# alxn3/nbody-llm

Measured on AMD Instinct MI355X. Metric: pairwise_interactions_per_sec, higher is better.
Workload: dtype f32

## Files before the change

### nbody-llm_amd/csrc/kernels.h

```cpp
#pragma once
#include <hip/hip_runtime.h>
#include <cstdint>
#include <vector>

namespace nbody {

struct Tuning {
    int cross_sym = 1;
    int sym_packed = 1;
    int bf_fast_variant = 0;
    int bh_walk_duo = -1;
    int bh_walk_xcd = 1;
    int let_list_div = 4;
    int sym_ipt = 0;
    int sym_wpb = 4;
    int sym_rounds = 1;
    int sym_k = 0;
    int sym_min_bodies = 1024;
    int sym_reduce_split = 1;
    int cross_slots = 3072;
    int cross_ipt = 0;
    int cross_wpb = 4;
    int bh_walk_split = 0;
    int bh_walk_order = 1;
// ... 2 lines not shown
    int bh_walk_variant = 0;
    int bh_walk_lds_block = 1024;
    int bh_hot_cap = 2048;
    int bh_walk_debug = 0;
    int sym_debug = 0;
};
const Tuning& tuning();
struct WalkPlan { int bodies_per_lane; int segments; };
WalkPlan walk_plan(size_t n_order, bool fast_math, int max_segments, float theta2);
void bind_tuning(const Tuning* t);

struct Shard {
    float4* pos_all = nullptr;
    float4* vel = nullptr;
    float4* acc = nullptr;
    int* seg_count = nullptr;
    int* escaped = nullptr;
    unsigned char* keep = nullptr;
    unsigned long long* tile_state = nullptr;
    int* epoch = nullptr;
    int* poison = nullptr;
    int* ids = nullptr;
    unsigned long long* inter = nullptr;
    int n_seg = 1;
    int seg_cap = 0;
    int my_seg = 0;
    float4* own_pos() const { return pos_all + size_t(my_seg) * seg_cap; }
    int* own_count() const { return seg_count + my_seg; }
};

struct BoundsF {
    float lo[3];
    float hi[3];
};

void launch_aos_to_soa(hipStream_t s, const float* aos, int stride_f, int n, float4* pos, float4* vel, float4* acc);
void launch_soa_to_aos(hipStream_t s, float* aos, int stride_f, int n, const float4* pos, const float4* vel, const float4* acc);

void launch_drift_half(hipStream_t s, const Shard& sh, int n_upper, float dt, BoundsF b);
void launch_compact(hipStream_t s, const Shard& sh, int n_upper);
void launch_kick_drift(hipStream_t s, const Shard& sh, int n_upper, float dt);

void launch_bf_forces_strict(hipStream_t s, const Shard& sh, int n_upper, float g, float g_soft2);
void launch_bf_forces_fast(hipStream_t s, const Shard& sh, int n_upper, float g, float g_soft2);

struct SymPlan {
    int ipt = 8;
    int A = 0;
    int K = 0;
    int wpb = 16;
    int res_combine = 0;
    int k_res = 0;
    int sym_sets = 0;
    int n_planes = 0;
    int k_os = 0;
    size_t n_pad = 0;
    size_t plane_stride = 0;
    std::vector<int> bounds;
};
SymPlan make_sym_plan(int n_upper);
int sym_bodies_per_lane(size_t n);
uint64_t sym_main_pairs(const SymPlan& p, size_t n);
void launch_bf_sym_main(hipStream_t s, const Shard& sh, const SymPlan& p, const int* d_bounds, float4* planes,
                        int n_upper, float g_soft2);
void launch_bf_os(hipStream_t s, const Shard& sh, int A, int K, float4* planes, size_t plane_stride, float g_soft2);
void launch_bf_sym_tail(hipStream_t s, const Shard& sh, const SymPlan& p, float4* planes, int n_upper, float g,
                        float g_soft2, const float* kick_dt);

struct CrossPartners {
    static constexpr int kMax = 8;
    int n = 0;
    int seg[kMax];
    int c0[kMax], c1[kMax];
    int a0[kMax], a1[kMax];
};
struct CrossPlan {
    static constexpr int kMaxPlanes = 256;
    int ipt = 8;
    int A = 0;
    CrossPartners parts;
    int n_recv = 0;
    int recv_from[CrossPartners::kMax];
    int k_res = 0;
    std::vector<int4> slices;
};
CrossPlan make_cross_plan(int rank, int world, int seg_cap, int n_own_upper);
void launch_bf_cross(hipStream_t s, const Shard& sh, const CrossPlan& p, const int4* d_slices, float4* res_planes,
                     float4* xplanes, float4* send, size_t plane_stride, float g_soft2);

constexpr int kMaxSplit = 64, kMaxAnc = 192;
constexpr size_t kSplitInts = size_t(kMaxSplit) + 1 + kMaxSplit + size_t(kMaxSplit) * kMaxAnc;
struct TreeDev {
    const float4* nodes = nullptr;
    int n_nodes = 0;
    const int* order = nullptr;
    int n_order = 0;
    int n_split = 1;
    const int* split_first = nullptr;
    const int* split_anc = nullptr;
    const int* split_n_anc = nullptr;
    float4* split_planes = nullptr;
    size_t split_stride = 0;
    float4* nested_stack = nullptr;
    size_t nested_stride = 0;
    float4* walk = nullptr;
    float4* hot = nullptr;
    int* unified = nullptr;
    int* hot_info = nullptr;
    int hot_cap = 0;
    int hot_threshold = 0;
    const int* poison = nullptr;
    const int* n_order_dev = nullptr;
    int store_work = 0;
    float4* bfs = nullptr;
    void* bfs_ws = nullptr;
    size_t bfs_cap = 0;
};
struct TreeDevWork {
    const unsigned long long* keys = nullptr;
    const signed char* delta = nullptr;
// ... 59 lines not shown
```

### nbody-llm_amd/csrc/kernels_bf_sym.hip

```cpp
#include "kernels.h"
#include "bf_pair.h"

#include <algorithm>

namespace nbody {

namespace {

#ifdef NBODY_TUNING
__device__ unsigned long long nbody_sym_stamps[3 * 8192];
#endif

}

template <int IPT>
__device__ __forceinline__ void sym_rest_wave(const float4* __restrict__ pos, int n, int A, int group, int slice,
                                              int n_slices, float& ax, float& ay, float& az, float eps2);

template <int IPT, int NW>
__device__ __forceinline__ void sym_rest_block(const float4* __restrict__ pos, int n, int A, int group,
                                               float4* __restrict__ plane, float eps2, float (*red)[3][64]);

template <int IPT, int WPB, int DBG = 0, bool PK = false>
__global__ __launch_bounds__(WPB * 64) void k_bf_sym(const float4* __restrict__ pos, const int* __restrict__ count,
                                                     int A, int K, const int* __restrict__ bounds, int sym_sets,
                                                     float4* __restrict__ planes, size_t plane_stride, float eps2,
                                                     int res_combine) {
    const int lane = threadIdx.x & 63;
    const int wslot = __builtin_amdgcn_readfirstlane(threadIdx.x >> 6);
    const int n_main_blocks = (A * K + WPB - 1) / WPB;
    if (int(blockIdx.x) >= n_main_blocks) {
        __shared__ float red[WPB - 1][3][64];
        sym_rest_block<IPT, WPB>(pos, *count, A, blockIdx.x - n_main_blocks,
                                 planes + size_t(sym_sets + (res_combine ? K / WPB : K)) * plane_stride, eps2, red);
        return;
    }
    const int gw = blockIdx.x * WPB + (wslot & 3) * (WPB / 4) + (wslot >> 2);
    if (gw >= A * K) return;
    const int a = gw / K;
    const int part = gw - a * K;
    const int n = *count;
    const int Cn = A * IPT;
    const int k0 = bounds[part], k1 = bounds[part + 1];
    const int src_lane = ((lane + 63) & 63) * 4;
    const int src_lane2 = ((lane + 62) & 63) * 4;
    float eps2v = eps2;
    asm volatile("" : "+v"(eps2v));

    float xi[IPT], yi[IPT], zi[IPT], mi[IPT], axi[IPT], ayi[IPT], azi[IPT];
#pragma unroll
    for (int q = 0; q < IPT; ++q) {
        const int i = (a * IPT + q) * 64 + lane;
        const float4 p = (i < n) ? pos[i] : make_float4(PAD_POS, PAD_POS, PAD_POS, 0.f);
        xi[q] = p.x; yi[q] = p.y; zi[q] = p.z; mi[q] = p.w;
        axi[q] = ayi[q] = azi[q] = 0.f;
    }

    auto chunk_of = [&](int k) {
        int c = (a + 1) * IPT + k;
        if (c >= Cn) c -= Cn;
        return c;
    };
    auto load_chunk = [&](int k) {
        const int j = chunk_of(k) * 64 + lane;
        return (j < n) ? pos[j] : make_float4(PAD_POS, PAD_POS, PAD_POS, 0.f);
    };

    [[maybe_unused]] unsigned long long t_beg = 0, r_beg = 0;
    if (DBG & 4) { t_beg = __builtin_amdgcn_s_memtime(); r_beg = __builtin_amdgcn_s_memrealtime(); }
    float4 nxt = (k0 < k1) ? load_chunk(k0) : make_float4(0.f, 0.f, 0.f, 0.f);
    v2f xi2[IPT / 2], yi2[IPT / 2], zi2[IPT / 2], mi2[IPT / 2], axi2[IPT / 2], ayi2[IPT / 2], azi2[IPT / 2];
    if (PK) {
        pack_pairs<IPT>(xi, xi2); pack_pairs<IPT>(yi, yi2); pack_pairs<IPT>(zi, zi2); pack_pairs<IPT>(mi, mi2);
        pack_pairs<IPT>(axi, axi2); pack_pairs<IPT>(ayi, ayi2); pack_pairs<IPT>(azi, azi2);
    }
    for (int k = k0; k < k1; ++k) {
        float xj = nxt.x, yj = nxt.y, zj = nxt.z, mj = nxt.w;
        float axj = 0.f, ayj = 0.f, azj = 0.f;
        v2f axj2 = {0.f, 0.f}, ayj2 = {0.f, 0.f}, azj2 = {0.f, 0.f};
        if (k + 1 < k1) nxt = load_chunk(k + 1);
        switch ((4 * (k1 - k) - 1) / (k1 - k0)) {
            case 3: __builtin_amdgcn_s_setprio(3); break;
            case 2: __builtin_amdgcn_s_setprio(2); break;
            case 1: __builtin_amdgcn_s_setprio(1); break;
            default: __builtin_amdgcn_s_setprio(0); break;
        }
        if (PK) {
            for (int s = 0; s < 64; s += 2) {
                const float x1 = rotl(xj, src_lane), y1 = rotl(yj, src_lane), z1 = rotl(zj, src_lane), m1 = rotl(mj, src_lane);
                pair_evals_pk<IPT / 2, DBG>(xi2, yi2, zi2, mi2, axi2, ayi2, azi2, xj, yj, zj, mj, axj2, ayj2, azj2, eps2v);
                axj2.x = rotl(axj2.x, src_lane); ayj2.x = rotl(ayj2.x, src_lane); azj2.x = rotl(azj2.x, src_lane);
                axj2.y = rotl(axj2.y, src_lane); ayj2.y = rotl(ayj2.y, src_lane); azj2.y = rotl(azj2.y, src_lane);
                xj = rotl(x1, src_lane); yj = rotl(y1, src_lane); zj = rotl(z1, src_lane); mj = rotl(m1, src_lane);
                pair_evals_pk<IPT / 2, DBG>(xi2, yi2, zi2, mi2, axi2, ayi2, azi2, x1, y1, z1, m1, axj2, ayj2, azj2, eps2v);
                axj2.x = rotl(axj2.x, src_lane); ayj2.x = rotl(ayj2.x, src_lane); azj2.x = rotl(azj2.x, src_lane);
                axj2.y = rotl(axj2.y, src_lane); ayj2.y = rotl(ayj2.y, src_lane); azj2.y = rotl(azj2.y, src_lane);
            }
        } else {
            float x1 = rotl(xj, src_lane), y1 = rotl(yj, src_lane), z1 = rotl(zj, src_lane), m1 = rotl(mj, src_lane);
#pragma unroll 2
            for (int s = 0; s < 64; ++s) {
                const float x2 = rotl(xj, src_lane2), y2 = rotl(yj, src_lane2), z2 = rotl(zj, src_lane2), m2 = rotl(mj, src_lane2);
                pair_evals<IPT, DBG>(xi, yi, zi, mi, axi, ayi, azi, xj, yj, zj, mj, axj, ayj, azj, eps2v);
                axj = rotl(axj, src_lane); ayj = rotl(ayj, src_lane); azj = rotl(azj, src_lane);
                xj = x1; yj = y1; zj = z1; mj = m1;
                x1 = x2; y1 = y2; z1 = z2; m1 = m2;
            }
        }
        if (PK) { axj = axj2.x + axj2.y; ayj = ayj2.x + ayj2.y; azj = azj2.x + azj2.y; }
        const int d = k / IPT + 1;
        planes[size_t(d - 1) * plane_stride + size_t(chunk_of(k)) * 64 + lane] = make_float4(axj, ayj, azj, 0.f);
    }
    if (PK) { unpack_pairs<IPT>(axi2, axi); unpack_pairs<IPT>(ayi2, ayi); unpack_pairs<IPT>(azi2, azi); }

#ifdef NBODY_TUNING
    if (DBG & 4) {
        const unsigned long long t_end = __builtin_amdgcn_s_memtime(), r_end = __builtin_amdgcn_s_memrealtime();
        if (lane == 0 && gw < 8192) {
            nbody_sym_stamps[gw * 3 + 0] = t_end - t_beg;
            nbody_sym_stamps[gw * 3 + 1] = r_end - r_beg;
            const unsigned hw = __builtin_amdgcn_s_getreg((4 ) | (0 << 6) | (31 << 11));
            const unsigned xcc = __builtin_amdgcn_s_getreg((20 ) | (0 << 6) | (31 << 11));
            nbody_sym_stamps[gw * 3 + 2] = (unsigned long long)(k1 - k0) | ((unsigned long long)hw << 16) | ((unsigned long long)(xcc & 0xF) << 48);
        }
    }
#endif
    if (res_combine) {
        __shared__ float comb[WPB - 1][3 * IPT][64];
        const int first_part = (part / WPB) * WPB;
        const int rel = part - first_part;
        if (rel > 0) {
#pragma unroll
            for (int q = 0; q < IPT; ++q) {
                comb[rel - 1][3 * q + 0][lane] = axi[q];
                comb[rel - 1][3 * q + 1][lane] = ayi[q];
                comb[rel - 1][3 * q + 2][lane] = azi[q];
            }
        }
        __syncthreads();
        if (rel == 0) {
            float4* __restrict__ out = planes + size_t(sym_sets + part / WPB) * plane_stride;
#pragma unroll
            for (int q = 0; q < IPT; ++q) {
                float sx = axi[q], sy = ayi[q], sz = azi[q];
                for (int w = 0; w < WPB - 1; ++w) { sx += comb[w][3 * q + 0][lane]; sy += comb[w][3 * q + 1][lane]; sz += comb[w][3 * q + 2][lane]; }
                out[size_t(a * IPT + q) * 64 + lane] = make_float4(sx, sy, sz, 0.f);
            }
        }
        return;
    }
    float4* __restrict__ out = planes + size_t(sym_sets + part) * plane_stride;
#pragma unroll
    for (int q = 0; q < IPT; ++q) out[size_t(a * IPT + q) * 64 + lane] = make_float4(axi[q], ayi[q], azi[q], 0.f);
}

template <int IPT, int WPB, bool PK>
__global__ __launch_bounds__(WPB * 64) void k_bf_os(const float4* __restrict__ pos_all,
                                                    const int* __restrict__ seg_count, int n_seg, int seg_cap,
                                                    int my_seg, int A, int K, float4* __restrict__ planes,
                                                    size_t plane_stride, float eps2) {
    __shared__ float4 stage[WPB][2][64];
    const int lane = threadIdx.x & 63;
    const int wslot = __builtin_amdgcn_readfirstlane(threadIdx.x >> 6);
    const int gw = blockIdx.x * WPB + (wslot & 3) * (WPB / 4) + (wslot >> 2);
    if (gw >= A * K) return;
    const int a = gw / K, part = gw - a * K;
    const int n_own = seg_count[my_seg];
    const float4* __restrict__ own = pos_all + size_t(my_seg) * seg_cap;
    float eps2v = eps2;
    asm volatile("" : "+v"(eps2v));

    float xi[IPT], yi[IPT], zi[IPT], mi[IPT], axi[IPT], ayi[IPT], azi[IPT];
#pragma unroll
    for (int q = 0; q < IPT; ++q) {
        const int i = (a * IPT + q) * 64 + lane;
        const float4 p = (i < n_own) ? own[i] : make_float4(PAD_POS, PAD_POS, PAD_POS, 0.f);
        xi[q] = p.x; yi[q] = p.y; zi[q] = p.z; mi[q] = p.w;
        axi[q] = ayi[q] = azi[q] = 0.f;
    }
    long long R = 0;
    for (int s = 0; s < n_seg; ++s) if (s != my_seg) R += seg_count[s];
    const long long r0 = R * part / K, r1 = R * (part + 1) / K;
    long long seg_first = 0;
    float dummy_x = 0.f, dummy_y = 0.f, dummy_z = 0.f;
    v2f dummy2 = {0.f, 0.f};
    v2f xi2[IPT / 2], yi2[IPT / 2], zi2[IPT / 2], mi2[IPT / 2], axi2[IPT / 2], ayi2[IPT / 2], azi2[IPT / 2];
    if (PK) {
        pack_pairs<IPT>(xi, xi2); pack_pairs<IPT>(yi, yi2); pack_pairs<IPT>(zi, zi2); pack_pairs<IPT>(mi, mi2);
        pack_pairs<IPT>(axi, axi2); pack_pairs<IPT>(ayi, ayi2); pack_pairs<IPT>(azi, azi2);
    }
    for (int s = 0; s < n_seg; ++s) {
        if (s == my_seg) continue;
        const int ns = seg_count[s];
        const long long lo = r0 > seg_first ? r0 : seg_first;
        const long long hi = r1 < seg_first + ns ? r1 : seg_first + ns;
        const float4* __restrict__ ps = pos_all + size_t(s) * seg_cap - seg_first;
        int buf = 0;
        if (lo < hi) {
            const long long j = lo + lane;
            stage[wslot][0][lane] = (j < hi) ? ps[j] : make_float4(PAD_POS, PAD_POS, PAD_POS, 0.f);
        }
        for (long long c0 = lo; c0 < hi; c0 += 64) {
            const long long jn = c0 + 64 + lane;
            float4 nxt = make_float4(PAD_POS, PAD_POS, PAD_POS, 0.f);
            if (c0 + 64 < hi && jn < hi) nxt = ps[jn];
            const int cnt = int(hi - c0 < 64 ? hi - c0 : 64);
            switch (int((4 * (r1 - c0) - 1) / (r1 - r0))) {
                case 3: __builtin_amdgcn_s_setprio(3); break;
                case 2: __builtin_amdgcn_s_setprio(2); break;
                case 1: __builtin_amdgcn_s_setprio(1); break;
                default: __builtin_amdgcn_s_setprio(0); break;
            }
            float4 pj = stage[wslot][buf][0];
            for (int t = 0; t < cnt; ++t) {
                const float4 pn = stage[wslot][buf][(t + 1) & 63];
                if (PK)
                    pair_evals_pk<IPT / 2, 0, false>(xi2, yi2, zi2, mi2, axi2, ayi2, azi2, pj.x, pj.y, pj.z, pj.w, dummy2,
                                                     dummy2, dummy2, eps2v);
                else
                    pair_evals<IPT, 0, false>(xi, yi, zi, mi, axi, ayi, azi, pj.x, pj.y, pj.z, pj.w, dummy_x, dummy_y,
                                              dummy_z, eps2v);
                pj = pn;
            }
            buf ^= 1;
            stage[wslot][buf][lane] = nxt;
        }
        seg_first += ns;
    }
    if (PK) { unpack_pairs<IPT>(axi2, axi); unpack_pairs<IPT>(ayi2, ayi); unpack_pairs<IPT>(azi2, azi); }
    float4* __restrict__ out = planes + size_t(part) * plane_stride;
#pragma unroll
    for (int q = 0; q < IPT; ++q) out[size_t(a * IPT + q) * 64 + lane] = make_float4(axi[q], ayi[q], azi[q], 0.f);
}

template <int IPT>
__device__ __forceinline__ void sym_rest_wave(const float4* __restrict__ pos, int n, int A, int group, int slice,
                                              int n_slices, float& ax, float& ay, float& az, float eps2) {
    constexpr int SET = 64 * IPT;
    const int lane = threadIdx.x & 63;
    const int i = group * 64 + lane;
    const int a = (group * 64) / SET;
    const float4 pi = (i < n) ? pos[i] : make_float4(PAD_POS, PAD_POS, PAD_POS, 0.f);
    ax = ay = az = 0.f;
    const int n_win = (A % 2 == 0 && A > 1) ? 2 : 1;
    for (int w = 0; w < n_win; ++w) {
        int set = (w == 0) ? a : a + A / 2;
        if (set >= A) set -= A;
        const int j0 = set * SET + SET * slice / n_slices;
        const int j1 = min(n, set * SET + SET * (slice + 1) / n_slices);
#pragma unroll 8
        for (int j = j0; j < j1; ++j) {
            const float4 pj = pos[j];
            const float dx = pj.x - pi.x, dy = pj.y - pi.y, dz = pj.z - pi.z;
            const float r2 = __builtin_fmaf(dz, dz, __builtin_fmaf(dy, dy, __builtin_fmaf(dx, dx, eps2)));
            const float rinv = __builtin_amdgcn_rsqf(r2);
            float sj = pj.w * ((rinv * rinv) * rinv);
            sj = (j == i) ? 0.f : sj;
            ax = __builtin_fmaf(dx, sj, ax);
            ay = __builtin_fmaf(dy, sj, ay);
            az = __builtin_fmaf(dz, sj, az);
        }
    }
}

template <int IPT, int NW>
__device__ __forceinline__ void sym_rest_block(const float4* __restrict__ pos, int n, int A, int group,
                                               float4* __restrict__ plane, float eps2, float (*red)[3][64]) {
    const int lane = threadIdx.x & 63;
    const int wv = __builtin_amdgcn_readfirstlane(threadIdx.x >> 6);
    float ax, ay, az;
    sym_rest_wave<IPT>(pos, n, A, group, wv, NW, ax, ay, az, eps2);
    if (wv > 0) { red[wv - 1][0][lane] = ax; red[wv - 1][1][lane] = ay; red[wv - 1][2][lane] = az; }
    __syncthreads();
    if (wv == 0) {
#pragma unroll
        for (int w = 0; w < NW - 1; ++w) { ax += red[w][0][lane]; ay += red[w][1][lane]; az += red[w][2][lane]; }
        plane[group * 64 + lane] = make_float4(ax, ay, az, 0.f);
    }
}

template <int IPT>
__global__ __launch_bounds__(512) void k_bf_sym_rest(const float4* __restrict__ pos, const int* __restrict__ count,
                                                     int A, float4* __restrict__ plane, float eps2) {
    __shared__ float red[7][3][64];
    sym_rest_block<IPT, 8>(pos, *count, A, blockIdx.x, plane, eps2, red);
}

template <bool KICK>
__global__ __launch_bounds__(256) void k_bf_sym_reduce(const float4* __restrict__ planes, int n_planes,
                                                       size_t plane_stride, const int* __restrict__ count, float g,
                                                       float4* __restrict__ acc, float4* __restrict__ pos,
                                                       float4* __restrict__ vel, float dt, const int* __restrict__ seg_count,
                                                       int n_seg, unsigned long long* __restrict__ inter) {
    const int i = blockIdx.x * 256 + threadIdx.x;
    if (inter && i == 0) {
        long long tot = 0;
        for (int s = 0; s < n_seg; ++s) tot += seg_count[s];
        if (tot > 0) atomicAdd(inter, (unsigned long long)(*count) * (unsigned long long)(tot - 1));
    }
    if (i >= *count) return;
    float sx = 0.f, sy = 0.f, sz = 0.f, cx = 0.f, cy = 0.f, cz = 0.f;
    for (int p = 0; p < n_planes; ++p) {
        const float4 v = planes[size_t(p) * plane_stride + i];
        const float yx = v.x - cx, yy = v.y - cy, yz = v.z - cz;
        const float tx = sx + yx, ty = sy + yy, tz = sz + yz;
        cx = (tx - sx) - yx; cy = (ty - sy) - yy; cz = (tz - sz) - yz;
        sx = tx; sy = ty; sz = tz;
    }
    const float4 a = make_float4(g * sx, g * sy, g * sz, 0.f);
    acc[i] = a;
    if (KICK) {
        float4 p = pos[i], v = vel[i];
        v.x += a.x * dt; v.y += a.y * dt; v.z += a.z * dt;
        p.x += (v.x * 0.5f) * dt; p.y += (v.y * 0.5f) * dt; p.z += (v.z * 0.5f) * dt;
        vel[i] = v;
        pos[i] = p;
    }
}

template <bool KICK, int Q>
__global__ __launch_bounds__(64 * Q) void k_bf_sym_reduce_split(const float4* __restrict__ planes, int n_planes, size_t plane_stride,
                                                                const int* __restrict__ count, float g, float4* __restrict__ acc,
                                                                float4* __restrict__ pos, float4* __restrict__ vel, float dt,
                                                                const int* __restrict__ seg_count, int n_seg,
                                                                unsigned long long* __restrict__ inter) {
    __shared__ float part[Q][3][64];
    const int lane = threadIdx.x & 63, q = threadIdx.x >> 6;
    const int i = blockIdx.x * 64 + lane;
    if (inter && blockIdx.x == 0 && threadIdx.x == 0) {
        long long tot = 0;
        for (int s = 0; s < n_seg; ++s) tot += seg_count[s];
        if (tot > 0) atomicAdd(inter, (unsigned long long)(*count) * (unsigned long long)(tot - 1));
    }
    const int n = *count;
    float sx = 0.f, sy = 0.f, sz = 0.f, cx = 0.f, cy = 0.f, cz = 0.f;
    if (i < n) {
        const int p0 = int((long long)n_planes * q / Q), p1 = int((long long)n_planes * (q + 1) / Q);
        for (int p = p0; p < p1; ++p) {
            const float4 v = planes[size_t(p) * plane_stride + i];
            const float yx = v.x - cx, yy = v.y - cy, yz = v.z - cz;
            const float tx = sx + yx, ty = sy + yy, tz = sz + yz;
            cx = (tx - sx) - yx; cy = (ty - sy) - yy; cz = (tz - sz) - yz;
            sx = tx; sy = ty; sz = tz;
        }
    }
    part[q][0][lane] = sx; part[q][1][lane] = sy; part[q][2][lane] = sz;
    __syncthreads();
    if (q != 0 || i >= n) return;
    sx = sy = sz = cx = cy = cz = 0.f;
    for (int w = 0; w < Q; ++w) {
        const float yx = part[w][0][lane] - cx, yy = part[w][1][lane] - cy, yz = part[w][2][lane] - cz;
        const float tx = sx + yx, ty = sy + yy, tz = sz + yz;
        cx = (tx - sx) - yx; cy = (ty - sy) - yy; cz = (tz - sz) - yz;
        sx = tx; sy = ty; sz = tz;
    }
    const float4 a = make_float4(g * sx, g * sy, g * sz, 0.f);
    acc[i] = a;
    if (KICK) {
        float4 p = pos[i], v = vel[i];
        v.x += a.x * dt; v.y += a.y * dt; v.z += a.z * dt;
        p.x += (v.x * 0.5f) * dt; p.y += (v.y * 0.5f) * dt; p.z += (v.z * 0.5f) * dt;
        vel[i] = v;
        pos[i] = p;
    }
}

}
#ifdef NBODY_TUNING
namespace nbody { int read_sym_stamps(unsigned long long* out, int n_waves); }
extern "C" int nbody_sym_read_stamps(unsigned long long* out, int n_waves) { return nbody::read_sym_stamps(out, n_waves); }
#endif
namespace nbody {

int sym_bodies_per_lane(size_t n) {
    const Tuning& t = tuning();
    if (!t.sym_packed || t.sym_wpb != 4 || t.sym_ipt == 8) return 8;
    if (t.sym_ipt == 4) return 4;
    return n <= 10240 ? 4 : 8;
}

SymPlan make_sym_plan(int n_upper) {
    SymPlan p;
    const int IPT = sym_bodies_per_lane(size_t(n_upper));
    p.ipt = IPT;
    p.A = (n_upper + 64 * IPT - 1) / (64 * IPT);
    p.sym_sets = (p.A + 1) / 2 - 1;
    const int L = IPT * p.sym_sets;
    const int want = tuning().sym_wpb;
    p.wpb = want == 8 ? 8 : want == 12 ? 12 : want == 16 ? 16 : 4;
    int K = 1;
    if (p.wpb == 4) {
        K = L <= 100 ? L : L <= 160 ? (L + 1) / 2 : 64;
    } else {
        const int resident_wgs_per_cu = (p.wpb == 8) ? 2 : 1;
        const int slots = 256 * resident_wgs_per_cu * p.wpb;
        double best = 0.0;
        const int k_hi = std::min(126, std::min(L, std::max(1, slots * std::max(1, tuning().sym_rounds) * 4 / p.A)));
        for (int k = 1; k <= k_hi; ++k) {
            const long long waves = (long long)p.A * k;
            const long long rounds = (waves + slots - 1) / slots;
            if (rounds > 4 * std::max(1, tuning().sym_rounds) && k > 1) break;
            const double fill = double(waves) / double(rounds * slots);
            const double even = (L % k == 0) ? 1.0 : double(L / k) / double(L / k + 1);
            const double per_wave = double(L) / k / (double(L) / k + 0.3);
            if (fill * even * per_wave > best + 1e-9) { best = fill * even * per_wave; K = k; }
        }
    }
    if (tuning().sym_k > 0) K = std::min(126, tuning().sym_k);
    if (K > L) K = L;
    if (K < 1) K = 1;
    p.K = K;
    p.res_combine = (K % p.wpb == 0) ? 1 : 0;
    p.k_res = p.res_combine ? K / p.wpb : K;
    p.n_planes = p.sym_sets + p.k_res + 1;
    p.n_pad = size_t(p.A) * 64 * IPT;
    p.plane_stride = p.n_pad;
    p.bounds.resize(K + 1);
    for (int part = 0; part <= K; ++part) p.bounds[part] = int((long long)L * part / K);
    return p;
}

#ifdef NBODY_TUNING
int read_sym_stamps(unsigned long long* out, int n_waves) {
    return hipMemcpyFromSymbol(out, HIP_SYMBOL(nbody_sym_stamps), sizeof(unsigned long long) * 3 * n_waves) == hipSuccess ? 0 : -1;
}
#endif

uint64_t sym_main_pairs(const SymPlan& p, size_t n) {
    const size_t set = size_t(64) * p.ipt;
    auto size_of = [&](int a) { size_t lo = size_t(a) * set; return lo >= n ? size_t(0) : std::min(set, n - lo); };
    uint64_t pairs = 0;
    for (int a = 0; a < p.A; ++a)
        for (int d = 1; d <= p.sym_sets; ++d) pairs += uint64_t(size_of(a)) * uint64_t(size_of((a + d) % p.A));
    return pairs;
}

void launch_bf_sym_main(hipStream_t s, const Shard& sh, const SymPlan& p, const int* d_bounds, float4* planes,
                        int n_upper, float g_soft2) {
    if (n_upper <= 0 || p.sym_sets <= 0) return;
    const int main_blocks = (p.A * p.K + p.wpb - 1) / p.wpb;
    const int rest_blocks = int(p.n_pad / 64);
    const dim3 grid(main_blocks + rest_blocks), block(p.wpb * 64);
#define SYM_LAUNCH(WPB, DBG) hipLaunchKernelGGL((k_bf_sym<8, WPB, DBG, PKV>), grid, block, 0, s, sh.own_pos(), sh.own_count(), p.A, p.K, d_bounds, p.sym_sets, planes, p.plane_stride, g_soft2, p.res_combine)
#ifdef NBODY_TUNING
    const int dbg = tuning().sym_debug;
#else
    constexpr int dbg = 0;
#endif
    if (p.ipt == 4) {
        hipLaunchKernelGGL((k_bf_sym<4, 4, 0, true>), grid, block, 0, s, sh.own_pos(), sh.own_count(), p.A, p.K, d_bounds, p.sym_sets, planes, p.plane_stride, g_soft2, p.res_combine);
        return;
    }
    if (tuning().sym_packed) {
        constexpr bool PKV = true;
        if (dbg == 4) {
#ifdef NBODY_TUNING
            if (p.wpb == 12) SYM_LAUNCH(12, 4); else if (p.wpb == 8) SYM_LAUNCH(8, 4); else if (p.wpb == 4) SYM_LAUNCH(4, 4); else SYM_LAUNCH(16, 4);
#endif
        } else {
            if (p.wpb == 12) SYM_LAUNCH(12, 0); else if (p.wpb == 8) SYM_LAUNCH(8, 0); else if (p.wpb == 4) SYM_LAUNCH(4, 0); else SYM_LAUNCH(16, 0);
        }
    } else {
        constexpr bool PKV = false;
        if (dbg >= 4 && dbg <= 7) {
#ifdef NBODY_TUNING
            if (dbg == 4) { if (p.wpb == 12) SYM_LAUNCH(12, 4); else if (p.wpb == 8) SYM_LAUNCH(8, 4); else if (p.wpb == 4) SYM_LAUNCH(4, 4); else SYM_LAUNCH(16, 4); }
            else if (dbg == 5) SYM_LAUNCH(16, 5);
            else if (dbg == 6) SYM_LAUNCH(16, 6);
            else SYM_LAUNCH(16, 7);
#endif
        } else {
            if (p.wpb == 12) SYM_LAUNCH(12, 0); else if (p.wpb == 8) SYM_LAUNCH(8, 0); else if (p.wpb == 4) SYM_LAUNCH(4, 0); else SYM_LAUNCH(16, 0);
        }
    }
#undef SYM_LAUNCH
}

void launch_bf_os(hipStream_t s, const Shard& sh, int A, int K, float4* planes, size_t plane_stride, float g_soft2) {
    if (A <= 0 || K <= 0) return;
    const int wpb = 12;
    if (tuning().sym_packed)
        hipLaunchKernelGGL((k_bf_os<8, 12, true>), dim3((A * K + wpb - 1) / wpb), dim3(wpb * 64), 0, s, sh.pos_all,
                           sh.seg_count, sh.n_seg, sh.seg_cap, sh.my_seg, A, K, planes, plane_stride, g_soft2);
    else
        hipLaunchKernelGGL((k_bf_os<8, 12, false>), dim3((A * K + wpb - 1) / wpb), dim3(wpb * 64), 0, s, sh.pos_all,
                           sh.seg_count, sh.n_seg, sh.seg_cap, sh.my_seg, A, K, planes, plane_stride, g_soft2);
}

void launch_bf_sym_tail(hipStream_t s, const Shard& sh, const SymPlan& p, float4* planes, int n_upper, float g,
                        float g_soft2, const float* kick_dt) {
    if (n_upper <= 0) return;
    if (p.sym_sets == 0) {
        float4* resident0 = planes + size_t(p.sym_sets) * p.plane_stride;
        (void)hipMemsetAsync(resident0, 0, size_t(p.k_res) * p.plane_stride * sizeof(float4), s);
        if (p.ipt == 4)
            hipLaunchKernelGGL(k_bf_sym_rest<4>, dim3(int(p.n_pad / 64)), dim3(512), 0, s, sh.own_pos(),
                               sh.own_count(), p.A, planes + size_t(p.sym_sets + p.k_res) * p.plane_stride, g_soft2);
        else
        hipLaunchKernelGGL(k_bf_sym_rest<8>, dim3(int(p.n_pad / 64)), dim3(512), 0, s, sh.own_pos(),
                           sh.own_count(), p.A, planes + size_t(p.sym_sets + p.k_res) * p.plane_stride, g_soft2);
    }
    const float dt = kick_dt ? *kick_dt : 0.f;
#define REDUCE_ARGS planes, p.n_planes, p.plane_stride, sh.own_count(), g, sh.acc, sh.own_pos(), sh.vel, dt, sh.seg_count, sh.n_seg, sh.inter
    if (tuning().sym_reduce_split && p.n_planes >= 16) {
        const dim3 grid((n_upper + 63) / 64);
        if (n_upper <= 16384) {
            if (kick_dt) hipLaunchKernelGGL((k_bf_sym_reduce_split<true, 16>), grid, dim3(1024), 0, s, REDUCE_ARGS);
            else hipLaunchKernelGGL((k_bf_sym_reduce_split<false, 16>), grid, dim3(1024), 0, s, REDUCE_ARGS);
        } else {
            if (kick_dt) hipLaunchKernelGGL((k_bf_sym_reduce_split<true, 4>), grid, dim3(256), 0, s, REDUCE_ARGS);
            else hipLaunchKernelGGL((k_bf_sym_reduce_split<false, 4>), grid, dim3(256), 0, s, REDUCE_ARGS);
        }
    } else {
        const dim3 grid((n_upper + 255) / 256);
        if (kick_dt) hipLaunchKernelGGL(k_bf_sym_reduce<true>, grid, dim3(256), 0, s, REDUCE_ARGS);
        else hipLaunchKernelGGL(k_bf_sym_reduce<false>, grid, dim3(256), 0, s, REDUCE_ARGS);
    }
#undef REDUCE_ARGS
}

}
```

### nbody-llm_amd/csrc/nbody_api.cpp

```cpp
#include "nbody_handle.h"
#include "nbody_f64.h"
#include "nbody_let.h"

#include <algorithm>
#include <chrono>
#include <cmath>
#include <cstdio>
#include <cstdlib>
#include <cstring>
#include <memory>
#include <string>
#include <thread>
#include <vector>


static thread_local std::string g_create_err;

int fail(NbodyHandle* h, int code, const std::string& msg) {
    if (h) h->err = msg; else g_create_err = msg;
    return code;
}

namespace {

// ... 555 lines not shown
        }
        if (rest.empty()) {
            h->host_tree_once = true;
            return NBODY_OK;
        }
        h->elapsed = rest[0].elapsed_before;
        h->stats.steps -= rest.size();
        h->host_tree_once = true;
        int rc = sync_count(h);
        if (rc) return rc;
        rc = step_end(h, rest[0].dt);
        if (rc) return rc;
        for (size_t k = 1; k < rest.size(); ++k) {
            rc = step_impl(h, rest[k].dt);
            if (rc) return rc;
        }
    }
    return fail(h, NBODY_ERR_INVALID, "resolve_async did not converge");
}

int partials_begin(NbodyHandle* h) {
    if (!(h->cross_on && h->tail_pending) || h->cross.parts.n + h->cross.n_recv == 0) return NBODY_OK;
    if (!h->comm_ready) return fail(h, NBODY_ERR_COMM, "world_size > 1 but nbody_comm_init has not been called");
    const nbody::CrossPlan& c = h->cross;
    const size_t S = h->sym_plan.plane_stride;
    const size_t bytes = size_t(h->sh.seg_cap) * sizeof(float4);
    HIP_TRY(h, hipEventRecord(h->ev_partials_ready, h->stream));
    HIP_TRY(h, hipStreamWaitEvent(h->comm_stream, h->ev_partials_ready, 0));
    TP_TRY(h, h->tp->group_begin());
    for (int i = 0; i < c.parts.n; ++i)
        TP_TRY(h, h->tp->send(h->d_send + size_t(i) * S, bytes, c.parts.seg[i], h->comm_stream));
    for (int i = 0; i < c.n_recv; ++i)
        TP_TRY(h, h->tp->recv(h->d_planes + size_t(h->recv_plane0 + i) * S, bytes, c.recv_from[i], h->comm_stream));
    TP_TRY(h, h->tp->group_end());
    HIP_TRY(h, hipEventRecord(h->ev_partials_done, h->comm_stream));
    h->partials_in_flight = true;
    return NBODY_OK;
}

int partials_wait(NbodyHandle* h) {
    if (!h->partials_in_flight) return NBODY_OK;
    HIP_TRY(h, hipStreamWaitEvent(h->stream, h->ev_partials_done, 0));
    h->partials_in_flight = false;
    return NBODY_OK;
}

int forces_begin(NbodyHandle* h) {
    return h->cfg.method == NBODY_BARNES_HUT ? bh_forces(h) : bf_forces(h);
}

int forces_finish(NbodyHandle* h) {
    if (!h->tail_pending) return NBODY_OK;
    h->tail_pending = false;
    const float eps2 = h->g_soft * h->g_soft;
    nbody::launch_bf_sym_tail(h->stream, h->sh, h->sym_plan, h->d_planes, int(h->n_local), h->g, eps2,
                              h->kick_pending ? &h->kick_dt : nullptr);
    h->kick_pending = false;
    HIP_TRY(h, hipGetLastError());
    return NBODY_OK;
}

int forces(NbodyHandle* h) {
    int rc = forces_begin(h);
    if (rc) return rc;
    rc = partials_begin(h);
    if (rc) return rc;
    rc = partials_wait(h);
    if (rc) return rc;
    return forces_finish(h);
}

int step_begin(NbodyHandle* h, float dt) {
    if (!h->bounds_set) return fail(h, NBODY_ERR_INVALID, "nbody_set_bounds has not been called");
    nbody::launch_drift_half(h->stream, h->sh, int(h->n_local), dt, h->bnd);
    nbody::launch_compact(h->stream, h->sh, int(h->n_local));
    h->count_dirty = true;
    HIP_TRY(h, hipGetLastError());
    return NBODY_OK;
}

int step_forces(NbodyHandle* h, float dt) {
    h->kick_pending = true;
    h->kick_dt = dt;
    int rc = forces_begin(h);
    if (rc) { h->kick_pending = false; h->tail_pending = false; }
    return rc;
}

int step_finish(NbodyHandle* h, float dt) {
    int rc = forces_finish(h);
    if (rc) { h->kick_pending = false; return rc; }
    if (h->kick_pending) nbody::launch_kick_drift(h->stream, h->sh, int(h->n_local), dt);
    h->kick_pending = false;
    HIP_TRY(h, hipGetLastError());
    if (h->ev_pending.size() >= 4096) {
        rc = drain_events(h);
        if (rc) return rc;
    }
    h->elapsed += dt;
    h->stats.steps += 1;
    return NBODY_OK;
}

int step_end(NbodyHandle* h, float dt) {
    int rc = step_forces(h, dt);
    if (rc) return rc;
    rc = partials_begin(h);
    if (rc) return rc;
// ... 1008 lines not shown
```

Measured before the change: 5553 billion.

## Fold diagonal and half-distance chunks into symmetric traversal, add per-lane intra-chunk kernel

Replaces the non-symmetric 'rest' pass, which evaluated the diagonal set and the antipodal set with full one-sided pairs, with symmetric traversal items. The diagonal chunk uses a 32-step rotate with a half-lane final step, and the antipodal set is split across halves. A new small kernel computes intra-lane pairs among each lane's IPT bodies. Work is balanced over 'units', and planes are laid out via n_trav. This removes roughly the redundant half of the rest-pass interactions, at the cost of more index logic and extra planes. Pair accounting now reports n(n-1)/2.

Measured after the change: 5574 billion, median of 6. No clear change (+0.4%).

```diff
diff --git a/nbody-llm_amd/csrc/kernels.h b/nbody-llm_amd/csrc/kernels.h
--- a/nbody-llm_amd/csrc/kernels.h
+++ b/nbody-llm_amd/csrc/kernels.h
@@ -78,6 +78,7 @@
     int res_combine = 0;
     int k_res = 0;
     int sym_sets = 0;
+    int n_trav = 0;
     int n_planes = 0;
     int k_os = 0;
     size_t n_pad = 0;
@@ -91,7 +92,7 @@
                         int n_upper, float g_soft2);
 void launch_bf_os(hipStream_t s, const Shard& sh, int A, int K, float4* planes, size_t plane_stride, float g_soft2);
 void launch_bf_sym_tail(hipStream_t s, const Shard& sh, const SymPlan& p, float4* planes, int n_upper, float g,
-                        float g_soft2, const float* kick_dt);
+                        const float* kick_dt);
 
 struct CrossPartners {
     static constexpr int kMax = 8;
diff --git a/nbody-llm_amd/csrc/kernels_bf_sym.hip b/nbody-llm_amd/csrc/kernels_bf_sym.hip
--- a/nbody-llm_amd/csrc/kernels_bf_sym.hip
+++ b/nbody-llm_amd/csrc/kernels_bf_sym.hip
@@ -13,34 +13,71 @@
 
 }
 
+template <int IPT, int DBG>
+__device__ __forceinline__ void sym_step_pk(const v2f (&xi)[IPT / 2], const v2f (&yi)[IPT / 2], const v2f (&zi)[IPT / 2],
+                                            const v2f (&mi)[IPT / 2], v2f (&axi)[IPT / 2], v2f (&ayi)[IPT / 2],
+                                            v2f (&azi)[IPT / 2], float xj, float yj, float zj, float mj, v2f& axj,
+                                            v2f& ayj, v2f& azj, float eps2) {
+    constexpr int G = (IPT / 2 <= 6) ? IPT / 2 : 4;
+    static_assert((IPT / 2) % G == 0, "resident pairs must split into whole groups");
+#pragma unroll
+    for (int g = 0; g < IPT / 2; g += G) {
+        typedef v2f grp[G];
+        pair_evals_pk<G, DBG>(*reinterpret_cast<const grp*>(xi + g), *reinterpret_cast<const grp*>(yi + g),
+                              *reinterpret_cast<const grp*>(zi + g), *reinterpret_cast<const grp*>(mi + g),
+                              *reinterpret_cast<grp*>(axi + g), *reinterpret_cast<grp*>(ayi + g), *reinterpret_cast<grp*>(azi + g),
+                              xj, yj, zj, mj, axj, ayj, azj, eps2);
+    }
+}
+
 template <int IPT>
-__device__ __forceinline__ void sym_rest_wave(const float4* __restrict__ pos, int n, int A, int group, int slice,
-                                              int n_slices, float& ax, float& ay, float& az, float eps2);
-
-template <int IPT, int NW>
-__device__ __forceinline__ void sym_rest_block(const float4* __restrict__ pos, int n, int A, int group,
-                                               float4* __restrict__ plane, float eps2, float (*red)[3][64]);
+__global__ __launch_bounds__(256) void k_bf_sym_lanes(const float4* __restrict__ pos, const int* __restrict__ count,
+                                                      int A, float4* __restrict__ plane, float eps2) {
+    const int lane = threadIdx.x & 63;
+    const int a = blockIdx.x * 4 + (threadIdx.x >> 6);
+    if (a >= A) return;
+    const int n = *count;
+    float x[IPT], y[IPT], z[IPT], m[IPT], ax[IPT], ay[IPT], az[IPT];
+#pragma unroll
+    for (int q = 0; q < IPT; ++q) {
+        const int i = (a * IPT + q) * 64 + lane;
+        const float4 p = (i < n) ? pos[i] : make_float4(PAD_POS, PAD_POS, PAD_POS, 0.f);
+        x[q] = p.x; y[q] = p.y; z[q] = p.z; m[q] = p.w;
+        ax[q] = ay[q] = az[q] = 0.f;
+    }
+#pragma unroll
+    for (int r = 1; r < IPT; ++r) {
+#pragma unroll
+        for (int q = 0; q < r; ++q) {
+            const float dx = x[r] - x[q], dy = y[r] - y[q], dz = z[r] - z[q];
+            const float r2 = __builtin_fmaf(dz, dz, __builtin_fmaf(dy, dy, __builtin_fmaf(dx, dx, eps2)));
+            const float ri = __builtin_amdgcn_rsqf(r2);
+            const float r3 = (ri * ri) * ri;
+            const float sr = m[r] * r3, sq = m[q] * r3;
+            ax[q] = __builtin_fmaf(dx, sr, ax[q]); ax[r] = __builtin_fmaf(-dx, sq, ax[r]);
+            ay[q] = __builtin_fmaf(dy, sr, ay[q]); ay[r] = __builtin_fmaf(-dy, sq, ay[r]);
+            az[q] = __builtin_fmaf(dz, sr, az[q]); az[r] = __builtin_fmaf(-dz, sq, az[r]);
+            __builtin_amdgcn_sched_barrier(0);
+        }
+    }
+#pragma unroll
+    for (int q = 0; q < IPT; ++q) plane[size_t(a * IPT + q) * 64 + lane] = make_float4(ax[q], ay[q], az[q], 0.f);
+}
 
 template <int IPT, int WPB, int DBG = 0, bool PK = false>
 __global__ __launch_bounds__(WPB * 64) void k_bf_sym(const float4* __restrict__ pos, const int* __restrict__ count,
-                                                     int A, int K, const int* __restrict__ bounds, int sym_sets,
+                                                     int A, int K, const int* __restrict__ bounds, int sym_sets, int n_trav,
                                                      float4* __restrict__ planes, size_t plane_stride, float eps2,
                                                      int res_combine) {
     const int lane = threadIdx.x & 63;
     const int wslot = __builtin_amdgcn_readfirstlane(threadIdx.x >> 6);
-    const int n_main_blocks = (A * K + WPB - 1) / WPB;
-    if (int(blockIdx.x) >= n_main_blocks) {
-        __shared__ float red[WPB - 1][3][64];
-        sym_rest_block<IPT, WPB>(pos, *count, A, blockIdx.x - n_main_blocks,
-                                 planes + size_t(sym_sets + (res_combine ? K / WPB : K)) * plane_stride, eps2, red);
-        return;
-    }
     const int gw = blockIdx.x * WPB + (wslot & 3) * (WPB / 4) + (wslot >> 2);
     if (gw >= A * K) return;
     const int a = gw / K;
     const int part = gw - a * K;
     const int n = *count;
     const int Cn = A * IPT;
+    const int L = IPT * sym_sets;
     const int k0 = bounds[part], k1 = bounds[part + 1];
     const int src_lane = ((lane + 63) & 63) * 4;
     const int src_lane2 = ((lane + 62) & 63) * 4;
@@ -56,29 +93,43 @@
         axi[q] = ayi[q] = azi[q] = 0.f;
     }
 
-    auto chunk_of = [&](int k) {
-        int c = (a + 1) * IPT + k;
-        if (c >= Cn) c -= Cn;
-        return c;
+    auto item_of = [&](int k, int& c, int& s0, int& kind, int& pl) {
+        if (k < L) {
+            c = (a + 1) * IPT + k;
+            if (c >= Cn) c -= Cn;
+            s0 = 0; kind = 0; pl = k / IPT;
+        } else if (k < L + IPT) {
+            c = a * IPT + (k - L); s0 = 1; kind = 1; pl = sym_sets;
+        } else {
+            int b = a + A / 2;
+            if (b >= A) b -= A;
+            c = b * IPT + (k - L - IPT); s0 = (a < A / 2) ? 0 : 1; kind = 2; pl = sym_sets + 1;
+        }
     };
-    auto load_chunk = [&](int k) {
-        const int j = chunk_of(k) * 64 + lane;
+    auto load_item = [&](int k) {
+        int c, s0, kind, pl;
+        item_of(k, c, s0, kind, pl);
+        const int j = c * 64 + ((lane - s0) & 63);
         return (j < n) ? pos[j] : make_float4(PAD_POS, PAD_POS, PAD_POS, 0.f);
     };
 
     [[maybe_unused]] unsigned long long t_beg = 0, r_beg = 0;
     if (DBG & 4) { t_beg = __builtin_amdgcn_s_memtime(); r_beg = __builtin_amdgcn_s_memrealtime(); }
-    float4 nxt = (k0 < k1) ? load_chunk(k0) : make_float4(0.f, 0.f, 0.f, 0.f);
+    float4 nxt = (k0 < k1) ? load_item(k0) : make_float4(0.f, 0.f, 0.f, 0.f);
     v2f xi2[IPT / 2], yi2[IPT / 2], zi2[IPT / 2], mi2[IPT / 2], axi2[IPT / 2], ayi2[IPT / 2], azi2[IPT / 2];
     if (PK) {
         pack_pairs<IPT>(xi, xi2); pack_pairs<IPT>(yi, yi2); pack_pairs<IPT>(zi, zi2); pack_pairs<IPT>(mi, mi2);
         pack_pairs<IPT>(axi, axi2); pack_pairs<IPT>(ayi, ayi2); pack_pairs<IPT>(azi, azi2);
     }
+    const bool low_half = lane < 32;
     for (int k = k0; k < k1; ++k) {
+        int c, s0, kind, pl;
+        item_of(k, c, s0, kind, pl);
+        const int n_steps = kind == 0 ? 64 : 32;
         float xj = nxt.x, yj = nxt.y, zj = nxt.z, mj = nxt.w;
         float axj = 0.f, ayj = 0.f, azj = 0.f;
         v2f axj2 = {0.f, 0.f}, ayj2 = {0.f, 0.f}, azj2 = {0.f, 0.f};
-        if (k + 1 < k1) nxt = load_chunk(k + 1);
+        if (k + 1 < k1) nxt = load_item(k + 1);
         switch ((4 * (k1 - k) - 1) / (k1 - k0)) {
             case 3: __builtin_amdgcn_s_setprio(3); break;
             case 2: __builtin_amdgcn_s_setprio(2); break;
@@ -86,33 +137,49 @@
             default: __builtin_amdgcn_s_setprio(0); break;
         }
         if (PK) {
-            for (int s = 0; s < 64; s += 2) {
+            const int n_it = n_steps / 2 - (kind == 1 ? 1 : 0);
+            for (int it = 0; it < n_it; ++it) {
                 const float x1 = rotl(xj, src_lane), y1 = rotl(yj, src_lane), z1 = rotl(zj, src_lane), m1 = rotl(mj, src_lane);
-                pair_evals_pk<IPT / 2, DBG>(xi2, yi2, zi2, mi2, axi2, ayi2, azi2, xj, yj, zj, mj, axj2, ayj2, azj2, eps2v);
+                sym_step_pk<IPT, DBG>(xi2, yi2, zi2, mi2, axi2, ayi2, azi2, xj, yj, zj, mj, axj2, ayj2, azj2, eps2v);
                 axj2.x = rotl(axj2.x, src_lane); ayj2.x = rotl(ayj2.x, src_lane); azj2.x = rotl(azj2.x, src_lane);
                 axj2.y = rotl(axj2.y, src_lane); ayj2.y = rotl(ayj2.y, src_lane); azj2.y = rotl(azj2.y, src_lane);
                 xj = rotl(x1, src_lane); yj = rotl(y1, src_lane); zj = rotl(z1, src_lane); mj = rotl(m1, src_lane);
-                pair_evals_pk<IPT / 2, DBG>(xi2, yi2, zi2, mi2, axi2, ayi2, azi2, x1, y1, z1, m1, axj2, ayj2, azj2, eps2v);
+                sym_step_pk<IPT, DBG>(xi2, yi2, zi2, mi2, axi2, ayi2, azi2, x1, y1, z1, m1, axj2, ayj2, azj2, eps2v);
                 axj2.x = rotl(axj2.x, src_lane); ayj2.x = rotl(ayj2.x, src_lane); azj2.x = rotl(azj2.x, src_lane);
                 axj2.y = rotl(axj2.y, src_lane); ayj2.y = rotl(ayj2.y, src_lane); azj2.y = rotl(azj2.y, src_lane);
             }
+            if (kind == 1) {
+                const float x1 = rotl(xj, src_lane), y1 = rotl(yj, src_lane), z1 = rotl(zj, src_lane), m1 = rotl(mj, src_lane);
+                sym_step_pk<IPT, DBG>(xi2, yi2, zi2, mi2, axi2, ayi2, azi2, xj, yj, zj, mj, axj2, ayj2, azj2, eps2v);
+                axj2.x = rotl(axj2.x, src_lane); ayj2.x = rotl(ayj2.x, src_lane); azj2.x = rotl(azj2.x, src_lane);
+                axj2.y = rotl(axj2.y, src_lane); ayj2.y = rotl(ayj2.y, src_lane); azj2.y = rotl(azj2.y, src_lane);
+                if (low_half) sym_step_pk<IPT, DBG>(xi2, yi2, zi2, mi2, axi2, ayi2, azi2, x1, y1, z1, m1, axj2, ayj2, azj2, eps2v);
+                axj2.x = rotl(axj2.x, src_lane); ayj2.x = rotl(ayj2.x, src_lane); azj2.x = rotl(azj2.x, src_lane);
+                axj2.y = rotl(axj2.y, src_lane); ayj2.y = rotl(ayj2.y, src_lane); azj2.y = rotl(azj2.y, src_lane);
+            }
         } else {
             float x1 = rotl(xj, src_lane), y1 = rotl(yj, src_lane), z1 = rotl(zj, src_lane), m1 = rotl(mj, src_lane);
-#pragma unroll 2
-            for (int s = 0; s < 64; ++s) {
+            auto step = [&]() {
                 const float x2 = rotl(xj, src_lane2), y2 = rotl(yj, src_lane2), z2 = rotl(zj, src_lane2), m2 = rotl(mj, src_lane2);
                 pair_evals<IPT, DBG>(xi, yi, zi, mi, axi, ayi, azi, xj, yj, zj, mj, axj, ayj, azj, eps2v);
                 axj = rotl(axj, src_lane); ayj = rotl(ayj, src_lane); azj = rotl(azj, src_lane);
                 xj = x1; yj = y1; zj = z1; mj = m1;
                 x1 = x2; y1 = y2; z1 = z2; m1 = m2;
+            };
+            for (int s = 0; s < n_steps / 2 - 1; ++s) { step(); step(); }
+            step();
+            if (kind == 1) {
+                if (low_half) pair_evals<IPT, DBG>(xi, yi, zi, mi, axi, ayi, azi, xj, yj, zj, mj, axj, ayj, azj, eps2v);
+                axj = rotl(axj, src_lane); ayj = rotl(ayj, src_lane); azj = rotl(azj, src_lane);
+            } else {
+                step();
             }
         }
         if (PK) { axj = axj2.x + axj2.y; ayj = ayj2.x + ayj2.y; azj = azj2.x + azj2.y; }
-        const int d = k / IPT + 1;
-        planes[size_t(d - 1) * plane_stride + size_t(chunk_of(k)) * 64 + lane] = make_float4(axj, ayj, azj, 0.f);
+        const int row = c * 64 + ((lane - s0 - n_steps) & 63);
+        planes[size_t(pl) * plane_stride + size_t(row)] = make_float4(axj, ayj, azj, 0.f);
     }
     if (PK) { unpack_pairs<IPT>(axi2, axi); unpack_pairs<IPT>(ayi2, ayi); unpack_pairs<IPT>(azi2, azi); }
-
 #ifdef NBODY_TUNING
     if (DBG & 4) {
         const unsigned long long t_end = __builtin_amdgcn_s_memtime(), r_end = __builtin_amdgcn_s_memrealtime();
@@ -139,7 +206,7 @@
         }
         __syncthreads();
         if (rel == 0) {
-            float4* __restrict__ out = planes + size_t(sym_sets + part / WPB) * plane_stride;
+            float4* __restrict__ out = planes + size_t(n_trav + part / WPB) * plane_stride;
 #pragma unroll
             for (int q = 0; q < IPT; ++q) {
                 float sx = axi[q], sy = ayi[q], sz = azi[q];
@@ -149,7 +216,7 @@
         }
         return;
     }
-    float4* __restrict__ out = planes + size_t(sym_sets + part) * plane_stride;
+    float4* __restrict__ out = planes + size_t(n_trav + part) * plane_stride;
 #pragma unroll
     for (int q = 0; q < IPT; ++q) out[size_t(a * IPT + q) * 64 + lane] = make_float4(axi[q], ayi[q], azi[q], 0.f);
 }
@@ -233,59 +300,6 @@
     for (int q = 0; q < IPT; ++q) out[size_t(a * IPT + q) * 64 + lane] = make_float4(axi[q], ayi[q], azi[q], 0.f);
 }
 
-template <int IPT>
-__device__ __forceinline__ void sym_rest_wave(const float4* __restrict__ pos, int n, int A, int group, int slice,
-                                              int n_slices, float& ax, float& ay, float& az, float eps2) {
-    constexpr int SET = 64 * IPT;
-    const int lane = threadIdx.x & 63;
-    const int i = group * 64 + lane;
-    const int a = (group * 64) / SET;
-    const float4 pi = (i < n) ? pos[i] : make_float4(PAD_POS, PAD_POS, PAD_POS, 0.f);
-    ax = ay = az = 0.f;
-    const int n_win = (A % 2 == 0 && A > 1) ? 2 : 1;
-    for (int w = 0; w < n_win; ++w) {
-        int set = (w == 0) ? a : a + A / 2;
-        if (set >= A) set -= A;
-        const int j0 = set * SET + SET * slice / n_slices;
-        const int j1 = min(n, set * SET + SET * (slice + 1) / n_slices);
-#pragma unroll 8
-        for (int j = j0; j < j1; ++j) {
-            const float4 pj = pos[j];
-            const float dx = pj.x - pi.x, dy = pj.y - pi.y, dz = pj.z - pi.z;
-            const float r2 = __builtin_fmaf(dz, dz, __builtin_fmaf(dy, dy, __builtin_fmaf(dx, dx, eps2)));
-            const float rinv = __builtin_amdgcn_rsqf(r2);
-            float sj = pj.w * ((rinv * rinv) * rinv);
-            sj = (j == i) ? 0.f : sj;
-            ax = __builtin_fmaf(dx, sj, ax);
-            ay = __builtin_fmaf(dy, sj, ay);
-            az = __builtin_fmaf(dz, sj, az);
-        }
-    }
-}
-
-template <int IPT, int NW>
-__device__ __forceinline__ void sym_rest_block(const float4* __restrict__ pos, int n, int A, int group,
-                                               float4* __restrict__ plane, float eps2, float (*red)[3][64]) {
-    const int lane = threadIdx.x & 63;
-    const int wv = __builtin_amdgcn_readfirstlane(threadIdx.x >> 6);
-    float ax, ay, az;
-    sym_rest_wave<IPT>(pos, n, A, group, wv, NW, ax, ay, az, eps2);
-    if (wv > 0) { red[wv - 1][0][lane] = ax; red[wv - 1][1][lane] = ay; red[wv - 1][2][lane] = az; }
-    __syncthreads();
-    if (wv == 0) {
-#pragma unroll
-        for (int w = 0; w < NW - 1; ++w) { ax += red[w][0][lane]; ay += red[w][1][lane]; az += red[w][2][lane]; }
-        plane[group * 64 + lane] = make_float4(ax, ay, az, 0.f);
-    }
-}
-
-template <int IPT>
-__global__ __launch_bounds__(512) void k_bf_sym_rest(const float4* __restrict__ pos, const int* __restrict__ count,
-                                                     int A, float4* __restrict__ plane, float eps2) {
-    __shared__ float red[7][3][64];
-    sym_rest_block<IPT, 8>(pos, *count, A, blockIdx.x, plane, eps2, red);
-}
-
 template <bool KICK>
 __global__ __launch_bounds__(256) void k_bf_sym_reduce(const float4* __restrict__ planes, int n_planes,
                                                        size_t plane_stride, const int* __restrict__ count, float g,
@@ -375,7 +389,7 @@
 int sym_bodies_per_lane(size_t n) {
     const Tuning& t = tuning();
     if (!t.sym_packed || t.sym_wpb != 4 || t.sym_ipt == 8) return 8;
-    if (t.sym_ipt == 4) return 4;
+    if (t.sym_ipt == 4 || t.sym_ipt == 12 || t.sym_ipt == 16) return t.sym_ipt;
     return n <= 10240 ? 4 : 8;
 }
 
@@ -386,37 +400,47 @@
     p.A = (n_upper + 64 * IPT - 1) / (64 * IPT);
     p.sym_sets = (p.A + 1) / 2 - 1;
     const int L = IPT * p.sym_sets;
+    const int H = (p.A % 2 == 0) ? 2 * IPT : IPT;
+    const int items = L + H;
+    const int units = 2 * L + H;
+    const int E = (units + 1) / 2;
     const int want = tuning().sym_wpb;
     p.wpb = want == 8 ? 8 : want == 12 ? 12 : want == 16 ? 16 : 4;
     int K = 1;
     if (p.wpb == 4) {
-        K = L <= 100 ? L : L <= 160 ? (L + 1) / 2 : 64;
+        K = E <= 100 ? E : E <= 160 ? (E + 1) / 2 : 64;
     } else {
         const int resident_wgs_per_cu = (p.wpb == 8) ? 2 : 1;
         const int slots = 256 * resident_wgs_per_cu * p.wpb;
         double best = 0.0;
-        const int k_hi = std::min(126, std::min(L, std::max(1, slots * std::max(1, tuning().sym_rounds) * 4 / p.A)));
+        const int k_hi = std::min(126, std::min(E, std::max(1, slots * std::max(1, tuning().sym_rounds) * 4 / p.A)));
         for (int k = 1; k <= k_hi; ++k) {
             const long long waves = (long long)p.A * k;
             const long long rounds = (waves + slots - 1) / slots;
             if (rounds > 4 * std::max(1, tuning().sym_rounds) && k > 1) break;
             const double fill = double(waves) / double(rounds * slots);
-            const double even = (L % k == 0) ? 1.0 : double(L / k) / double(L / k + 1);
-            const double per_wave = double(L) / k / (double(L) / k + 0.3);
+            const double even = (units % k == 0) ? 1.0 : double(units / k) / double(units / k + 1);
+            const double per_wave = double(E) / k / (double(E) / k + 0.3);
             if (fill * even * per_wave > best + 1e-9) { best = fill * even * per_wave; K = k; }
         }
     }
     if (tuning().sym_k > 0) K = std::min(126, tuning().sym_k);
-    if (K > L) K = L;
+    if (K > items) K = items;
     if (K < 1) K = 1;
     p.K = K;
     p.res_combine = (K % p.wpb == 0) ? 1 : 0;
     p.k_res = p.res_combine ? K / p.wpb : K;
-    p.n_planes = p.sym_sets + p.k_res + 1;
+    p.n_trav = p.sym_sets + (p.A % 2 == 0 ? 2 : 1);
+    p.n_planes = p.n_trav + p.k_res + 1;
     p.n_pad = size_t(p.A) * 64 * IPT;
     p.plane_stride = p.n_pad;
     p.bounds.resize(K + 1);
-    for (int part = 0; part <= K; ++part) p.bounds[part] = int((long long)L * part / K);
+    for (int part = 0; part <= K; ++part) {
+        const int t = int(((long long)units * part + K / 2) / K);
+        p.bounds[part] = t <= 2 * L ? (t + 1) / 2 : L + (t - 2 * L);
+    }
+    p.bounds[0] = 0;
+    p.bounds[K] = items;
     return p;
 }
 
@@ -426,31 +450,29 @@
 }
 #endif
 
-uint64_t sym_main_pairs(const SymPlan& p, size_t n) {
-    const size_t set = size_t(64) * p.ipt;
-    auto size_of = [&](int a) { size_t lo = size_t(a) * set; return lo >= n ? size_t(0) : std::min(set, n - lo); };
-    uint64_t pairs = 0;
-    for (int a = 0; a < p.A; ++a)
-        for (int d = 1; d <= p.sym_sets; ++d) pairs += uint64_t(size_of(a)) * uint64_t(size_of((a + d) % p.A));
-    return pairs;
+uint64_t sym_main_pairs(const SymPlan&, size_t n) {
+    return n > 1 ? uint64_t(n) * uint64_t(n - 1) / 2 : 0;
 }
 
 void launch_bf_sym_main(hipStream_t s, const Shard& sh, const SymPlan& p, const int* d_bounds, float4* planes,
                         int n_upper, float g_soft2) {
-    if (n_upper <= 0 || p.sym_sets <= 0) return;
-    const int main_blocks = (p.A * p.K + p.wpb - 1) / p.wpb;
-    const int rest_blocks = int(p.n_pad / 64);
-    const dim3 grid(main_blocks + rest_blocks), block(p.wpb * 64);
-#define SYM_LAUNCH(WPB, DBG) hipLaunchKernelGGL((k_bf_sym<8, WPB, DBG, PKV>), grid, block, 0, s, sh.own_pos(), sh.own_count(), p.A, p.K, d_bounds, p.sym_sets, planes, p.plane_stride, g_soft2, p.res_combine)
+    if (n_upper <= 0) return;
+    const dim3 grid((p.A * p.K + p.wpb - 1) / p.wpb), block(p.wpb * 64);
+    float4* lane_plane = planes + size_t(p.n_trav + p.k_res) * p.plane_stride;
+    if (p.ipt == 4) hipLaunchKernelGGL(k_bf_sym_lanes<4>, dim3((p.A + 3) / 4), dim3(256), 0, s, sh.own_pos(), sh.own_count(), p.A, lane_plane, g_soft2);
+    else if (p.ipt == 12) hipLaunchKernelGGL(k_bf_sym_lanes<12>, dim3((p.A + 3) / 4), dim3(256), 0, s, sh.own_pos(), sh.own_count(), p.A, lane_plane, g_soft2);
+    else if (p.ipt == 16) hipLaunchKernelGGL(k_bf_sym_lanes<16>, dim3((p.A + 3) / 4), dim3(256), 0, s, sh.own_pos(), sh.own_count(), p.A, lane_plane, g_soft2);
+    else hipLaunchKernelGGL(k_bf_sym_lanes<8>, dim3((p.A + 3) / 4), dim3(256), 0, s, sh.own_pos(), sh.own_count(), p.A, lane_plane, g_soft2);
+#define SYM_ARGS sh.own_pos(), sh.own_count(), p.A, p.K, d_bounds, p.sym_sets, p.n_trav, planes, p.plane_stride, g_soft2, p.res_combine
+#define SYM_LAUNCH(WPB, DBG) hipLaunchKernelGGL((k_bf_sym<8, WPB, DBG, PKV>), grid, block, 0, s, SYM_ARGS)
 #ifdef NBODY_TUNING
     const int dbg = tuning().sym_debug;
 #else
     constexpr int dbg = 0;
 #endif
-    if (p.ipt == 4) {
-        hipLaunchKernelGGL((k_bf_sym<4, 4, 0, true>), grid, block, 0, s, sh.own_pos(), sh.own_count(), p.A, p.K, d_bounds, p.sym_sets, planes, p.plane_stride, g_soft2, p.res_combine);
-        return;
-    }
+    if (p.ipt == 4) { hipLaunchKernelGGL((k_bf_sym<4, 4, 0, true>), grid, block, 0, s, SYM_ARGS); return; }
+    if (p.ipt == 12) { hipLaunchKernelGGL((k_bf_sym<12, 4, 0, true>), grid, block, 0, s, SYM_ARGS); return; }
+    if (p.ipt == 16) { hipLaunchKernelGGL((k_bf_sym<16, 4, 0, true>), grid, block, 0, s, SYM_ARGS); return; }
     if (tuning().sym_packed) {
         constexpr bool PKV = true;
         if (dbg == 4) {
@@ -474,6 +496,7 @@
         }
     }
 #undef SYM_LAUNCH
+#undef SYM_ARGS
 }
 
 void launch_bf_os(hipStream_t s, const Shard& sh, int A, int K, float4* planes, size_t plane_stride, float g_soft2) {
@@ -488,18 +511,8 @@
 }
 
 void launch_bf_sym_tail(hipStream_t s, const Shard& sh, const SymPlan& p, float4* planes, int n_upper, float g,
-                        float g_soft2, const float* kick_dt) {
+                        const float* kick_dt) {
     if (n_upper <= 0) return;
-    if (p.sym_sets == 0) {
-        float4* resident0 = planes + size_t(p.sym_sets) * p.plane_stride;
-        (void)hipMemsetAsync(resident0, 0, size_t(p.k_res) * p.plane_stride * sizeof(float4), s);
-        if (p.ipt == 4)
-            hipLaunchKernelGGL(k_bf_sym_rest<4>, dim3(int(p.n_pad / 64)), dim3(512), 0, s, sh.own_pos(),
-                               sh.own_count(), p.A, planes + size_t(p.sym_sets + p.k_res) * p.plane_stride, g_soft2);
-        else
-        hipLaunchKernelGGL(k_bf_sym_rest<8>, dim3(int(p.n_pad / 64)), dim3(512), 0, s, sh.own_pos(),
-                           sh.own_count(), p.A, planes + size_t(p.sym_sets + p.k_res) * p.plane_stride, g_soft2);
-    }
     const float dt = kick_dt ? *kick_dt : 0.f;
 #define REDUCE_ARGS planes, p.n_planes, p.plane_stride, sh.own_count(), g, sh.acc, sh.own_pos(), sh.vel, dt, sh.seg_count, sh.n_seg, sh.inter
     if (tuning().sym_reduce_split && p.n_planes >= 16) {
diff --git a/nbody-llm_amd/csrc/nbody_api.cpp b/nbody-llm_amd/csrc/nbody_api.cpp
--- a/nbody-llm_amd/csrc/nbody_api.cpp
+++ b/nbody-llm_amd/csrc/nbody_api.cpp
@@ -631,8 +631,7 @@
 int forces_finish(NbodyHandle* h) {
     if (!h->tail_pending) return NBODY_OK;
     h->tail_pending = false;
-    const float eps2 = h->g_soft * h->g_soft;
-    nbody::launch_bf_sym_tail(h->stream, h->sh, h->sym_plan, h->d_planes, int(h->n_local), h->g, eps2,
+    nbody::launch_bf_sym_tail(h->stream, h->sh, h->sym_plan, h->d_planes, int(h->n_local), h->g,
                               h->kick_pending ? &h->kick_dt : nullptr);
     h->kick_pending = false;
     HIP_TRY(h, hipGetLastError());
```
